# weikaolun/horovod-distributed-example

Hardware: AMD Instinct MI355X
Metric: images/sec (whole node) + scaling efficiency, ResNet-50 bf16 at 1/2/4/8 MI355X (higher is better)
Workload: dtype bf16; 1 GPU; model=ResNet-50, global_batch=2048, per_gpu_batch=2048, image=224, parallelism=dp1, optimizer=mivod FusedSGD via DistributedOptimizer, compression=none, transport=local, hip_graph=False

## Files before the change

### csrc/kernels/mv_conv.hip

```cpp
#include "mv_common.h"
#include "mv_conv.h"
#include "mv_gemm.h"

#include <algorithm>
#include <cstdlib>

namespace mv {
namespace conv {

typedef __bf16 bf16x8 __attribute__((ext_vector_type(8)));
typedef float f32x4v __attribute__((ext_vector_type(4)));
typedef uint32_t u32x2 __attribute__((ext_vector_type(2)));

constexpr int BK = 64;

__device__ __attribute__((aligned(16))) uint32_t g_zero[32];

__device__ __forceinline__ f32x4v mfma(const bf16x8& a, const bf16x8& b, const f32x4v& c) {
  return __builtin_amdgcn_mfma_f32_16x16x32_bf16(a, b, c, 0, 0, 0);
}
__device__ __forceinline__ int swz(int row, int ch) { return row * BK + ((ch ^ (row & 7)) << 3); }
__device__ __forceinline__ float round_bf16(float x) { return (float)(__bf16)x; }

__device__ __forceinline__ int remap(int bid, int nwg) {
  const int xcd = bid & 7, q = nwg >> 3, r = nwg & 7;
  const int base = xcd < r ? xcd * (q + 1) : r * (q + 1) + (xcd - r) * q;
  return base + (bid >> 3);
}

__device__ __forceinline__ void glds16(const void* src, __bf16* lds_wave_base) {
  __builtin_amdgcn_global_load_lds((const __attribute__((address_space(1))) void*)src,
                                   (__attribute__((address_space(3))) void*)lds_wave_base, 16, 0,
                                   0);
}

__device__ __forceinline__ void blds16(__amdgpu_buffer_rsrc_t rs, uint32_t off, __bf16* lds_wave_base) {
  __builtin_amdgcn_raw_ptr_buffer_load_lds(
      rs, (__attribute__((address_space(3))) void*)lds_wave_base, 16, off, 0, 0, 0);
}

struct Geo {
  int H, W, C, Ho, Wo, K, st;
  int64_t M;
  int ks = 3;
  int ph = 0, pw = 0;
  const __bf16* dy2 = nullptr;
  int k1 = 0;
  uint32_t xbytes = 0, wbytes = 0;
  int dy2x = 0;
};

template <int A_CH>
struct RowInfo {
  uint32_t addr[A_CH];
  uint32_t valid[A_CH];
};

template <int A_CH, int NT, bool DG = false>
__device__ __forceinline__ void row_info(const Geo& g, const __bf16* X, int64_t m0, int tid,
                                         int sc, RowInfo<A_CH>& ri) {
#pragma unroll
  for (int i = 0; i < A_CH; ++i) {
    const int64_t m = m0 + i * (NT / 8) + (tid >> 3);
    ri.valid[i] = 0;
    ri.addr[i] = 0;
    if (DG && m < g.M) {
      const uint32_t hw = (uint32_t)(g.Ho * g.Wo);
      const int rem = (int)((uint32_t)m % hw);
      const int ci = (int)((uint32_t)rem / (uint32_t)g.Wo), cj = rem - ci * g.Wo;
      const bool r1 = ci + 1 < g.Ho, c1 = cj + 1 < g.Wo;
      ri.valid[i] = 1u | (c1 ? 2u : 0u) | (r1 ? 4u : 0u) | (r1 && c1 ? 8u : 0u);
      ri.addr[i] = (uint32_t)((m * g.C + sc * 8) * 2);
    } else if (m < g.M) {
      const uint32_t hw = (uint32_t)(g.Ho * g.Wo), m32 = (uint32_t)m;
      const int n = (int)(m32 / hw);
      const int rem = (int)(m32 - (uint32_t)n * hw);
      const int ho = (int)((uint32_t)rem / (uint32_t)g.Wo), wo = rem - ho * g.Wo;
      const int pad = g.ks >> 1;
      const int hi0 = ho * g.st - pad, wi0 = wo * g.st - pad;
      uint32_t v = 0;
#pragma unroll
      for (int r = 0; r < 3; ++r)
#pragma unroll
        for (int s = 0; s < 3; ++s) {
          const bool ok = r < g.ks && s < g.ks && (unsigned)(hi0 + r) < (unsigned)g.H &&
                          (unsigned)(wi0 + s) < (unsigned)g.W;
          v |= (ok ? 1u : 0u) << (r * g.ks + s);
        }
      ri.valid[i] = v;
      ri.addr[i] = (uint32_t)(((((int64_t)n * g.H + hi0) * g.W + wi0) * g.C + sc * 8) * 2);
    }
  }
}

template <int N>
__device__ __forceinline__ void wait_vm() {
  asm volatile("s_waitcnt vmcnt(%0)" ::"n"(N) : "memory");
}

__device__ __forceinline__ void raw_barrier() {
  asm volatile("" ::: "memory");
  __builtin_amdgcn_s_barrier();
  asm volatile("" ::: "memory");
}

template <int BM, int BN, int WM, int WN, int EPI, int NS = 3, bool DG = false>
__global__ __launch_bounds__(WM * WN * 64)
__attribute__((amdgpu_waves_per_eu((NS == 2 && WM * WN == 8) ? 4 : 1))) void conv3x3_kernel(
    const __bf16* __restrict__ X, const __bf16* __restrict__ Wt, __bf16* __restrict__ Y, Geo g,
    int ntn, int64_t ntm, const float* __restrict__ shift, float* __restrict__ partial,
    const __bf16* __restrict__ bnx, const float* __restrict__ bnvec) {
  constexpr bool STATS = EPI != 0;
  constexpr int NT = WM * WN * 64;
  constexpr int A_CH = BM * 8 / NT;
  constexpr int WTN = BN / WN, WTM = BM / WM;
  constexpr int TN = WTN / 16, TM = WTM / 16;
  constexpr int B_CH = BN * 8 / NT;
  constexpr int LPS = A_CH + B_CH;
  constexpr int STAGE = (BM + BN) * BK;
  static_assert(NS == 2 || NS == 3, "LDS ring: 2 slots (1 stage in flight, 2 workgroups per "
                                     "CU) or 3 slots (2 stages in flight)");
  __shared__ __attribute__((aligned(16))) __bf16 smem[NS * STAGE];

  const int tid = threadIdx.x, lane = tid & 63;
  const int wid = __builtin_amdgcn_readfirstlane(tid >> 6);
  const int wm = wid / WN, wn = wid % WN;
  const int t = remap(blockIdx.x, gridDim.x);
  const int nt = t % ntn;
  const int64_t stream = t / ntn, nstreams = gridDim.x / ntn;
  const int n0 = nt * BN;
  const int taps = g.ks * g.ks;
  const int csteps = g.C / BK, KT = (DG ? (1 + g.ph) * (1 + g.pw) : taps) * csteps;
  const bool cpow2 = (csteps & (csteps - 1)) == 0;
  const int cshift = __builtin_ctz((unsigned)csteps);
  const int64_t wrow = (int64_t)taps * g.C;
  const int sc = (tid & 7) ^ ((tid >> 3) & 7);

  uint32_t brow[B_CH];
#pragma unroll
  for (int i = 0; i < B_CH; ++i)
    brow[i] = (uint32_t)(((int64_t)(n0 + i * (NT / 8) + (tid >> 3)) * wrow + sc * 8) * 2);
  const __amdgpu_buffer_rsrc_t rsX =
      __builtin_amdgcn_make_buffer_rsrc((void*)X, (short)0, (int)g.xbytes, 0x00020000);
  const __amdgpu_buffer_rsrc_t rsW =
      __builtin_amdgcn_make_buffer_rsrc((void*)Wt, (short)0, (int)g.wbytes, 0x00020000);

  auto issue = [&](const RowInfo<A_CH>& ri, int kt, int buf) {
    int tap = cpow2 ? kt >> cshift : kt / csteps;
    const int c0 = (kt - tap * csteps) * BK;
    uint32_t offa, offb;
    if constexpr (DG) {
      const int tR = g.pw ? tap >> 1 : tap, tS = g.pw ? tap & 1 : 0;
      const int rr = g.ph ? 2 * tR : 1, ss = g.pw ? 2 * tS : 1;
      offa = (uint32_t)(((tR * g.Wo + tS) * g.C + c0) * 2);
      offb = (uint32_t)(((rr * 3 + ss) * g.C + c0) * 2);
      tap = 2 * tR + tS;
    } else {
      const int r = g.ks == 3 ? (tap * 11) >> 5 : tap / g.ks;
      const int s = tap - r * g.ks;
      offa = (uint32_t)(((r * g.W + s) * g.C + c0) * 2);
      offb = (uint32_t)((tap * g.C + c0) * 2);
    }
    __bf16* As = smem + buf * STAGE;
    __bf16* Bs = As + BM * BK;
#pragma unroll
    for (int i = 0; i < A_CH; ++i) {
      const uint32_t a = ((ri.valid[i] >> tap) & 1u) ? ri.addr[i] + offa : 0xFFFFFFF0u;
      blds16(rsX, a, As + (i * NT + wid * 64) * 8);
    }
#pragma unroll
    for (int i = 0; i < B_CH; ++i)
      blds16(rsW, brow[i] + offb, Bs + (i * NT + wid * 64) * 8);
  };

  const int gq = lane >> 4, rl = lane & 15;
  float sh[EPI == 1 ? TN : 1][4], s1[TN][4], s2[TN][4];
#pragma unroll
  for (int a = 0; a < TN; ++a)
#pragma unroll
    for (int r = 0; r < 4; ++r) {
      const int col = n0 + wn * WTN + a * 16 + 4 * gq + r;
      if constexpr (EPI == 1) sh[a][r] = shift ? shift[col] : 0.f;
      s1[a][r] = 0.f;
      s2[a][r] = 0.f;
    }
  f32x4v acc[TN][TM];
#pragma unroll
  for (int a = 0; a < TN; ++a)
#pragma unroll
    for (int b = 0; b < TM; ++b) acc[a][b] = f32x4v{0.f, 0.f, 0.f, 0.f};

  int64_t mt = stream;
  if (mt < ntm) {
    RowInfo<A_CH> iri;
    row_info<A_CH, NT, DG>(g, X, mt * BM, tid, sc, iri);
    int64_t imt = mt;
    int ikt = 0;
    int islot = 0;
    issue(iri, 0, 0);
    auto issue_next = [&]() -> bool {
      int k2 = ikt + 1;
      int64_t m2 = imt;
      if (k2 == KT) { k2 = 0; m2 += nstreams; }
      if (m2 >= ntm) return false;
      if (m2 != imt) row_info<A_CH, NT, DG>(g, X, m2 * BM, tid, sc, iri);
      islot = islot + 1 == NS ? 0 : islot + 1;
      issue(iri, k2, islot);
      imt = m2;
      ikt = k2;
      return true;
    };
    bool ahead = NS == 3 ? issue_next() : false;
    int slot = 0;
    while (true) {
#pragma unroll
      for (int a = 0; a < TN; ++a)
#pragma unroll
        for (int b = 0; b < TM; ++b) acc[a][b] = f32x4v{0.f, 0.f, 0.f, 0.f};
      for (int kt = 0; kt < KT; ++kt) {
        if (NS == 3 && ahead) wait_vm<LPS>(); else wait_vm<0>();
        raw_barrier();
        ahead = issue_next();
        const __bf16* As = smem + slot * STAGE;
        const __bf16* Bs = As + BM * BK;
#pragma unroll
        for (int kk = 0; kk < BK / 32; ++kk) {
          const int ch = kk * 4 + gq;
          bf16x8 wf[TN], af[TM];
#pragma unroll
          for (int a = 0; a < TN; ++a)
            wf[a] = *reinterpret_cast<const bf16x8*>(Bs + swz(wn * WTN + a * 16 + rl, ch));
#pragma unroll
          for (int b = 0; b < TM; ++b)
            af[b] = *reinterpret_cast<const bf16x8*>(As + swz(wm * WTM + b * 16 + rl, ch));
#pragma unroll
          for (int a = 0; a < TN; ++a)
#pragma unroll
            for (int b = 0; b < TM; ++b) acc[a][b] = mfma(wf[a], af[b], acc[a][b]);
        }
        slot = slot + 1 == NS ? 0 : slot + 1;
      }
      const int64_t m0 = mt * BM;
#pragma unroll
      for (int b = 0; b < TM; ++b) {
        int64_t row = m0 + wm * WTM + b * 16 + rl;
        if (row < g.M) {
          if constexpr (DG) {
            const uint32_t hw = (uint32_t)(g.Ho * g.Wo), r32 = (uint32_t)row;
            const uint32_t n = r32 / hw, rem = r32 - n * hw;
            const uint32_t ci = rem / (uint32_t)g.Wo, cj = rem - ci * (uint32_t)g.Wo;
            row = ((int64_t)n * g.H + 2 * ci + g.ph) * g.W + 2 * cj + g.pw;
          }
#pragma unroll
          for (int a = 0; a < TN; ++a) {
            const f32x4v v = acc[a][b];
            const int col = n0 + wn * WTN + a * 16 + 4 * gq;
            if constexpr (EPI == 2) {
              const u32x2 xw = *reinterpret_cast<const u32x2*>(bnx + row * g.K + col);
              const float xv[4] = {__uint_as_float(xw[0] << 16), __uint_as_float(xw[0] & 0xffff0000u),
                                   __uint_as_float(xw[1] << 16), __uint_as_float(xw[1] & 0xffff0000u)};
              const float4 mu = *reinterpret_cast<const float4*>(bnvec + col);
              const float4 sc4 = *reinterpret_cast<const float4*>(bnvec + 2 * g.K + col);
              const float4 bi4 = *reinterpret_cast<const float4*>(bnvec + 3 * g.K + col);
              const float mus[4] = {mu.x, mu.y, mu.z, mu.w};
              const float scs[4] = {sc4.x, sc4.y, sc4.z, sc4.w};
              const float bis[4] = {bi4.x, bi4.y, bi4.z, bi4.w};
              float dv[4];
#pragma unroll
              for (int r = 0; r < 4; ++r) {
                const float d =
                    __builtin_fmaf(xv[r], scs[r], bis[r]) > 0.f ? round_bf16(v[r]) : 0.f;
                dv[r] = d;
                s1[a][r] += d;
                s2[a][r] += d * (xv[r] - mus[r]);
              }
              *reinterpret_cast<u32x2*>(Y + row * g.K + col) =
                  u32x2{cvt_pk_bf16(dv[0], dv[1]), cvt_pk_bf16(dv[2], dv[3])};
            } else {
              *reinterpret_cast<u32x2*>(Y + row * g.K + col) =
                  u32x2{cvt_pk_bf16(v[0], v[1]), cvt_pk_bf16(v[2], v[3])};
            }
            if (EPI == 1) {
#pragma unroll
              for (int r = 0; r < 4; ++r) {
                const float d = round_bf16(v[r]) - sh[a][r];
                s1[a][r] += d;
                s2[a][r] += d * d;
              }
            }
          }
        }
      }
      mt += nstreams;
      if (mt >= ntm) break;
    }
    wait_vm<0>();
    __syncthreads();
  }
  if (!STATS) return;
#pragma unroll
  for (int a = 0; a < TN; ++a)
#pragma unroll
    for (int r = 0; r < 4; ++r)
#pragma unroll
      for (int o = 1; o < 16; o <<= 1) {
        s1[a][r] += __shfl_xor(s1[a][r], o, kWave);
        s2[a][r] += __shfl_xor(s2[a][r], o, kWave);
      }
  __syncthreads();
  float* red = reinterpret_cast<float*>(smem);
  if (rl == 0) {
#pragma unroll
    for (int a = 0; a < TN; ++a)
#pragma unroll
      for (int r = 0; r < 4; ++r) {
        const int c = wn * WTN + a * 16 + 4 * gq + r;
        red[(0 * WM + wm) * BN + c] = s1[a][r];
        red[(1 * WM + wm) * BN + c] = s2[a][r];
      }
  }
  __syncthreads();
  if (stream >= ntm) return;
  for (int v = tid; v < 2 * BN; v += NT) {
    const int k = v / BN, c = v - k * BN;
    float acc_s = 0.f;
#pragma unroll
    for (int w = 0; w < WM; ++w) acc_s += red[(k * WM + w) * BN + c];
    partial[(stream * 2 + k) * g.K + n0 + c] = acc_s;
  }
}

template <int BN, bool STATS>
struct Cfg;
template <bool STATS>
struct Cfg<128, STATS> {
  static constexpr int BM = 128, WM = 2, WN = 2, NS = 2;
};
template <bool STATS>
struct Cfg<64, STATS> {
  static constexpr int BM = 256, WM = 4, WN = 2, NS = 2;
};

template <int BN, bool STATS, int EPI = STATS ? 1 : 0>
static const void* kernel_ptr() {
  using C = Cfg<BN, STATS>;
  return (const void*)&conv3x3_kernel<C::BM, BN, C::WM, C::WN, EPI, C::NS>;
}

template <int BN, bool STATS>
static int64_t streams_for(int64_t ntm, int ntn) {
  static int per = [] {
    int v = 0;
    if (hipOccupancyMaxActiveBlocksPerMultiprocessor(
            &v, kernel_ptr<BN, STATS>(), Cfg<BN, STATS>::WM * Cfg<BN, STATS>::WN * 64, 0) !=
            hipSuccess || v < 1)
      v = 1;
    return v;
  }();
  static int cus = [] {
    int dev = 0, v = 0;
    if (hipGetDevice(&dev) != hipSuccess ||
        hipDeviceGetAttribute(&v, hipDeviceAttributeMultiprocessorCount, dev) != hipSuccess || v < 1)
      v = 256;
    return v;
  }();
  int64_t s = (int64_t)cus * per / ntn;
  s = std::max<int64_t>(1, std::min(s, ntm));
  return s;
}

}
}

static int conv_bn_of(int K) { return K % 128 == 0 ? 128 : 64; }

static bool conv256_route(int K) { return K % 256 == 0 && K <= 2048; }

int64_t mv_conv3x3_partials(int64_t M, int K) {
  using namespace mv::conv;
  if (conv256_route(K)) return mv_gemm256_partials(M, K);
  if (conv_bn_of(K) == 128)
    return streams_for<128, true>((M + Cfg<128, true>::BM - 1) / Cfg<128, true>::BM, K / 128);
  return streams_for<64, true>((M + Cfg<64, true>::BM - 1) / Cfg<64, true>::BM, K / 64);
}

bool mv_conv3x3(const void* x, const void* w, void* y, int N, int H, int W, int C, int K,
                int stride, const float* shift, float* partial, hipStream_t st,
                const void* bn_x, const float* bn_vec) {
  return mv_conv_nhwc(x, w, y, N, H, W, C, K, 3, stride, shift, partial, st, bn_x, bn_vec);
}

bool mv_conv_nhwc(const void* x, const void* w, void* y, int N, int H, int W, int C, int K, int ks,
                  int stride, const float* shift, float* partial, hipStream_t st,
                  const void* bn_x, const float* bn_vec, const float* in_scale,
                  const float* in_bias) {
  using namespace mv::conv;
  if (C % 64 != 0 || K % 64 != 0 || (stride != 1 && stride != 2) || (ks != 1 && ks != 3))
    return false;
  if ((int64_t)N * H * W >= (int64_t(1) << 31)) return false;
  const bool bna = in_scale != nullptr;
  if (mv_conv64_supported(N, H, W, C, K, ks, stride)) {
    const int64_t M = (int64_t)N * H * W;
    int grid = partial ? (int)mv_conv3x3_partials(M, K) : 0;
    if (!partial) {
      int dev = 0, cus = 0;
      if (hipGetDevice(&dev) != hipSuccess ||
          hipDeviceGetAttribute(&cus, hipDeviceAttributeMultiprocessorCount, dev) != hipSuccess ||
          cus < 1)
        cus = 256;
      grid = cus;
    }
    return mv_conv64(x, w, y, N, H, W, shift, partial, grid, st, bn_x, bn_vec, in_scale,
                     in_bias);
  }
  if (bna) return false;
  if (conv256_route(K))
    return mv_conv256(x, w, y, N, H, W, C, K, ks, stride, shift, partial, bn_x, bn_vec, st);
  Geo g;
  g.ks = ks;
  g.H = H;
  g.W = W;
  g.C = C;
  g.K = K;
  g.st = stride;
  g.Ho = (H - 1) / stride + 1;
  g.Wo = (W - 1) / stride + 1;
  g.M = (int64_t)N * g.Ho * g.Wo;
  if ((int64_t)N * H * W * C * 2 >= (int64_t(1) << 32) - 16 ||
      (int64_t)K * ks * ks * C * 2 >= (int64_t(1) << 32) - 16)
    return false;
  g.xbytes = (uint32_t)((int64_t)N * H * W * C * 2);
  g.wbytes = (uint32_t)((int64_t)K * ks * ks * C * 2);
  const __bf16* X = (const __bf16*)x;
  const __bf16* Wt = (const __bf16*)w;
  __bf16* Y = (__bf16*)y;
  const __bf16* BX = (const __bf16*)bn_x;
  if (bn_x && !partial) return false;
#define MV_LAUNCH(BNV, ST)                                                                     \
  {                                                                                            \
    constexpr int BMV = Cfg<BNV, ST>::BM, WMV = Cfg<BNV, ST>::WM, WNV = Cfg<BNV, ST>::WN;      \
    constexpr int NSV = Cfg<BNV, ST>::NS;                                                      \
    const int64_t ntm = (g.M + BMV - 1) / BMV;                                                 \
    const int ntn = K / BNV;                                                                   \
    const int64_t ns = streams_for<BNV, ST>(ntm, ntn);                                         \
    if (BX)                                                                                    \
      hipLaunchKernelGGL((conv3x3_kernel<BMV, BNV, WMV, WNV, 2, NSV>), dim3((unsigned)(ns * ntn)),\
                         dim3(WMV * WNV * 64), 0, st, X, Wt, Y, g, ntn, ntm, shift, partial, BX, \
                         bn_vec);                                                              \
    else                                                                                       \
      hipLaunchKernelGGL((conv3x3_kernel<BMV, BNV, WMV, WNV, ST ? 1 : 0, NSV>),                  \
                         dim3((unsigned)(ns * ntn)), dim3(WMV * WNV * 64), 0, st, X, Wt, Y, g,   \
                         ntn, ntm, shift, partial, BX, bn_vec);                                \
  }
  if (conv_bn_of(K) == 128) {
    if (partial) MV_LAUNCH(128, true) else MV_LAUNCH(128, false)
  } else {
    if (partial) MV_LAUNCH(64, true) else MV_LAUNCH(64, false)
  }
#undef MV_LAUNCH
  return true;
}

namespace mv {
namespace conv {
struct TfTensor {
  const __bf16* src;
  __bf16* dst;
  int K, C, ks;
};
struct TfBlock {
  int t, tap, k0, c0;
};
__global__ __launch_bounds__(256) void transpose_filters_kernel(const TfTensor* __restrict__ ts,
                                                                const TfBlock* __restrict__ bl) {
  __shared__ __attribute__((aligned(16))) __bf16 tile[64][72];
  const TfBlock b = bl[blockIdx.x];
  const TfTensor tt = ts[b.t];
  const int ks = tt.ks, taps = ks * ks;
  const int r = b.tap / ks, s = b.tap - r * ks;
  const int ftap = (ks - 1 - r) * ks + (ks - 1 - s);
  typedef __bf16 bf16x8t __attribute__((ext_vector_type(8)));
  if (b.k0 + 64 <= tt.K && b.c0 + 64 <= tt.C && (tt.C & 7) == 0 && (tt.K & 7) == 0) {
    const int lr = threadIdx.x >> 3, l8 = (threadIdx.x & 7) * 8;
#pragma unroll
    for (int h = 0; h < 2; ++h) {
      const int i = lr + 32 * h;
      *reinterpret_cast<bf16x8t*>(&tile[i][l8]) = *reinterpret_cast<const bf16x8t*>(
          tt.src + ((int64_t)(b.k0 + i) * taps + ftap) * tt.C + b.c0 + l8);
    }
    __syncthreads();
#pragma unroll
    for (int h = 0; h < 2; ++h) {
      const int i = lr + 32 * h;
      bf16x8t v;
#pragma unroll
      for (int j = 0; j < 8; ++j) v[j] = tile[l8 + j][i];
      *reinterpret_cast<bf16x8t*>(tt.dst + ((int64_t)(b.c0 + i) * taps + b.tap) * tt.K + b.k0 +
                                  l8) = v;
    }
    return;
  }
  const int tx = threadIdx.x & 63, ty = threadIdx.x >> 6;
  for (int i = ty; i < 64; i += 4) {
    const int k = b.k0 + i, c = b.c0 + tx;
    tile[i][tx] = (k < tt.K && c < tt.C) ? tt.src[((int64_t)k * taps + ftap) * tt.C + c]
                                         : (__bf16)0.f;
  }
  __syncthreads();
  for (int i = ty; i < 64; i += 4) {
    const int c = b.c0 + i, k = b.k0 + tx;
    if (c < tt.C && k < tt.K) tt.dst[((int64_t)c * taps + b.tap) * tt.K + k] = tile[tx][i];
  }
}
}
}

int64_t mv_transpose_filters_blocks(const int* K, const int* C, const int* ks, int n) {
  int64_t nb = 0;
  for (int i = 0; i < n; ++i)
    nb += (int64_t)ks[i] * ks[i] * ((K[i] + 63) / 64) * ((C[i] + 63) / 64);
  return nb;
}

void mv_transpose_filters_table(const void* const* src, void* const* dst, const int* K,
                                const int* C, const int* ks, int n, void* host_image) {
  using namespace mv::conv;
  TfTensor* ts = reinterpret_cast<TfTensor*>(host_image);
  TfBlock* bl = reinterpret_cast<TfBlock*>(ts + n);
  int64_t j = 0;
  for (int i = 0; i < n; ++i) {
    ts[i] = TfTensor{(const __bf16*)src[i], (__bf16*)dst[i], K[i], C[i], ks[i]};
    for (int tap = 0; tap < ks[i] * ks[i]; ++tap)
      for (int k0 = 0; k0 < K[i]; k0 += 64)
        for (int c0 = 0; c0 < C[i]; c0 += 64) bl[j++] = TfBlock{i, tap, k0, c0};
  }
}

int64_t mv_transpose_filters_table_bytes(int n, int64_t blocks) {
  return (int64_t)n * (int64_t)sizeof(mv::conv::TfTensor) + blocks * (int64_t)sizeof(mv::conv::TfBlock);
}

void mv_transpose_filters(const void* table, int n, int64_t blocks, hipStream_t st) {
  using namespace mv::conv;
  const TfTensor* ts = reinterpret_cast<const TfTensor*>(table);
  const TfBlock* bl = reinterpret_cast<const TfBlock*>(ts + n);
  hipLaunchKernelGGL(transpose_filters_kernel, dim3((unsigned)blocks), dim3(256), 0, st, ts, bl);
}

bool mv_conv3x3_s2_dgrad_supported(int Nb, int H, int W, int C, int K) {
  if (mv_dgrad256_s2_supported(Nb, H, W, C, K)) return true;
  return Nb > 0 && H >= 2 && W >= 2 && !(H & 1) && !(W & 1) && C % 64 == 0 && K % 64 == 0 &&
         C > 0 && K > 0 && (int64_t)Nb * (H / 2) * (W / 2) * K * 2 < (int64_t(1) << 32) - 16 &&
         (int64_t)C * 9 * K * 2 < (int64_t(1) << 32) - 16 && (int64_t)Nb * H * W < (int64_t(1) << 31);
}

bool mv_conv3x3_s2_dgrad(const void* dy, const void* wt, void* dx, int Nb, int H, int W, int C,
                         int K, hipStream_t st) {
  using namespace mv::conv;
  if (mv_dgrad256_s2_supported(Nb, H, W, C, K))
    return mv_dgrad256_s2(dy, wt, dx, Nb, H, W, C, K, st);
  if (!mv_conv3x3_s2_dgrad_supported(Nb, H, W, C, K)) return false;
  Geo g;
  g.ks = 3;
  g.st = 2;
  g.H = H;
  g.W = W;
  g.C = K;
  g.K = C;
  g.Ho = H / 2;
  g.Wo = W / 2;
  g.M = (int64_t)Nb * g.Ho * g.Wo;
  g.xbytes = (uint32_t)(g.M * K * 2);
  g.wbytes = (uint32_t)((int64_t)C * 9 * K * 2);
  const __bf16* X = (const __bf16*)dy;
  const __bf16* Wt = (const __bf16*)wt;
  __bf16* Y = (__bf16*)dx;
#define MV_LAUNCH_DG(BNV)                                                                      \
  {                                                                                            \
    constexpr int BMV = Cfg<BNV, false>::BM, WMV = Cfg<BNV, false>::WM;                        \
    constexpr int WNV = Cfg<BNV, false>::WN, NSV = Cfg<BNV, false>::NS;                        \
    const int64_t ntm = (g.M + BMV - 1) / BMV;                                                 \
    const int ntn = C / BNV;                                                                   \
    const int64_t ns = streams_for<BNV, false>(ntm, ntn);                                      \
    hipLaunchKernelGGL((conv3x3_kernel<BMV, BNV, WMV, WNV, 0, NSV, true>),                      \
                       dim3((unsigned)(ns * ntn)), dim3(WMV * WNV * 64), 0, st, X, Wt, Y, g, ntn, \
                       ntm, nullptr, nullptr, nullptr, nullptr);                               \
  }
  for (int c = 3; c >= 0; --c) {
    g.ph = c >> 1;
    g.pw = c & 1;
    if (conv_bn_of(C) == 128) MV_LAUNCH_DG(128) else MV_LAUNCH_DG(64)
  }
#undef MV_LAUNCH_DG
  return true;
}

namespace mv {
// ... 542 lines not shown
```

### csrc/kernels/mv_conv64.hip

```cpp
#include "mv_common.h"
#include "mv_conv.h"

#include <type_traits>

namespace mv {
namespace conv64 {

typedef __bf16 bf16x8 __attribute__((ext_vector_type(8)));
typedef float f32x4v __attribute__((ext_vector_type(4)));
typedef uint32_t u32x2 __attribute__((ext_vector_type(2)));
typedef uint32_t u32x4 __attribute__((ext_vector_type(4)));

constexpr int kC = 64;
constexpr int kR = 8;
constexpr int kPR = kR + 2;
constexpr int kPW = 64;
constexpr int kThreads = 512;
constexpr int kTMW = 7;
constexpr int kTN = 2;
constexpr int kMaxW = kPW - 2;
constexpr int kMT = 4 * kTMW;
constexpr int kFilt = kC * 9 * kC;
constexpr int kPatchChunks = kPR * kPW * 8;
constexpr int kLoads = (kPatchChunks + kThreads - 1) / kThreads;

__device__ __forceinline__ f32x4v mfma(const bf16x8& a, const bf16x8& b, const f32x4v& c) {
  return __builtin_amdgcn_mfma_f32_16x16x32_bf16(a, b, c, 0, 0, 0);
}
__device__ __forceinline__ int fidx(int k, int tap, int c) {
  return ((k * 9 + tap) * 8 + (c ^ (k & 7))) * 8;
}
__device__ __forceinline__ int pidx(int row, int col, int c) {
  return ((row * kPW + col) * 8 + (c ^ (col & 7))) * 8;
}
__device__ __forceinline__ float round_bf16(float x) { return (float)(__bf16)x; }

struct Geo64 {
  int N, H, W;
  int hblocks;
  int64_t tiles;
};

__device__ __forceinline__ void bn_relu8(u32x4& v, const float (&sc)[8], const float (&bi)[8]) {
  uint32_t w[4] = {v[0], v[1], v[2], v[3]};
#pragma unroll
  for (int j = 0; j < 4; ++j) {
    const float lo = fmaxf(__builtin_fmaf(__uint_as_float(w[j] << 16), sc[2 * j], bi[2 * j]), 0.f);
    const float hi =
        fmaxf(__builtin_fmaf(__uint_as_float(w[j] & 0xffff0000u), sc[2 * j + 1], bi[2 * j + 1]), 0.f);
    w[j] = cvt_pk_bf16(lo, hi);
  }
  v = u32x4{w[0], w[1], w[2], w[3]};
}

template <int EPI>
__global__ __launch_bounds__(kThreads, 1) __attribute__((amdgpu_waves_per_eu(2, 2))) void conv64_kernel(
    const __bf16* __restrict__ X, const __bf16* __restrict__ Wt, __bf16* __restrict__ Y,
    Geo64 g, const float* __restrict__ shift, float* __restrict__ partial,
    const __bf16* __restrict__ bnx, const float* __restrict__ bnvec,
    const float* __restrict__ xsc, const float* __restrict__ xbi) {
  __shared__ __attribute__((aligned(16))) __bf16 lds[kFilt + kPR * kPW * kC];
  __bf16* fs = lds;
  __bf16* ps = lds + kFilt;
  const int tid = threadIdx.x, lane = tid & 63;
  const int wv = __builtin_amdgcn_readfirstlane(tid >> 6);
  const int nh = wv & 1, mg = wv >> 1;
  const int gq = lane >> 4, rl = lane & 15;
  const int W = g.W, H = g.H;

  for (int q = tid; q < kC * 9 * 8; q += kThreads) {
    const int k = q / 72, rem = q - k * 72, tap = rem >> 3, c = rem & 7;
    *reinterpret_cast<u32x4*>(fs + fidx(k, tap, c)) =
        *reinterpret_cast<const u32x4*>(Wt + (int64_t)q * 8);
  }

  int pbase[kTMW], pcol[kTMW];
#pragma unroll
  for (int b = 0; b < kTMW; ++b) {
    const int p = (mg * kTMW + b) * 16 + rl;
    const int r = p / W, c = p - r * W;
    const bool ok = r < kR;
    pbase[b] = ok ? (r * kPW + c) * 64 : 0;
    pcol[b] = ok ? c : 0;
  }

  static_assert(kThreads == 8 * kPW && kLoads == kPR, "one patch row per load");
  const int scol = tid >> 3, sch = tid & 7;
  const bool colok = scol >= 1 && scol - 1 < W;
  const int64_t coff = (int64_t)(scol - 1) * kC + sch * 8;
  const int soff = pidx(0, scol, sch);
  const bool bna = EPI != 2 && xsc != nullptr;
  float asc[8], abi[8];
#pragma unroll
  for (int j = 0; j < 8; ++j) {
    asc[j] = bna ? xsc[sch * 8 + j] : 0.f;
    abi[j] = bna ? xbi[sch * 8 + j] : 0.f;
  }
  u32x4 pre[kLoads];
  auto gload = [&](int64_t t) {
    const int n = (int)(t / g.hblocks), h0 = (int)(t - (int64_t)n * g.hblocks) * kR;
    const __bf16* img = X + (int64_t)n * H * W * kC;
#pragma unroll
    for (int i = 0; i < kLoads; ++i) {
      const int ih = h0 + i - 1;
      u32x4 v = {0u, 0u, 0u, 0u};
      if (colok && ih >= 0 && ih < H)
        v = *reinterpret_cast<const u32x4*>(img + (int64_t)ih * W * kC + coff);
      pre[i] = v;
    }
  };

  float s1[kTN][4], s2[kTN][4];
#pragma unroll
  for (int a = 0; a < kTN; ++a)
#pragma unroll
    for (int r = 0; r < 4; ++r) {
      s1[a][r] = 0.f;
      s2[a][r] = 0.f;
    }

  f32x4v acc[kTN][kTMW];
  auto epilogue = [&](int64_t tp) {
    const float* shp = shift;
    const float* bvp = bnvec;
    asm volatile("" : "+s"(shp));
    asm volatile("" : "+s"(bvp));
    const int n = (int)(tp / g.hblocks), h0 = (int)(tp - (int64_t)n * g.hblocks) * kR;
    float4 cv[EPI == 0 ? 1 : kTN][EPI == 2 ? 3 : 1];
    if constexpr (EPI != 0) {
#pragma unroll
      for (int a = 0; a < kTN; ++a) {
        const int col = nh * 32 + a * 16 + 4 * gq;
        if constexpr (EPI == 1) {
          cv[a][0] = shp ? *reinterpret_cast<const float4*>(shp + col) : float4{0.f, 0.f, 0.f, 0.f};
        } else {
          cv[a][0] = *reinterpret_cast<const float4*>(bvp + col);
          cv[a][1] = *reinterpret_cast<const float4*>(bvp + 2 * kC + col);
          cv[a][2] = *reinterpret_cast<const float4*>(bvp + 3 * kC + col);
        }
      }
    }
    const __bf16* ximg = bnx + (EPI == 2 ? (int64_t)n * H * W * kC : 0);
    __bf16* yimg = Y + (int64_t)n * H * W * kC;
    auto half = [&](auto b0c, auto b1c) {
      constexpr int B0 = decltype(b0c)::value, B1 = decltype(b1c)::value;
      int off[B1 - B0];
      bool ok[B1 - B0];
#pragma unroll
      for (int b = B0; b < B1; ++b) {
        const int p = (mg * kTMW + b) * 16 + rl;
        const int r = p / W;
        ok[b - B0] = r < kR && h0 + r < H;
        off[b - B0] = ((h0 + r) * W + (p - r * W)) * kC;
      }
      u32x2 xw[EPI == 2 ? B1 - B0 : 1][EPI == 2 ? kTN : 1];
      if constexpr (EPI == 2) {
#pragma unroll
        for (int b = B0; b < B1; ++b)
#pragma unroll
          for (int a = 0; a < kTN; ++a)
            xw[b - B0][a] = ok[b - B0] ? *reinterpret_cast<const u32x2*>(
                                             ximg + off[b - B0] + nh * 32 + a * 16 + 4 * gq)
                                       : u32x2{0u, 0u};
      }
#pragma unroll
      for (int b = B0; b < B1; ++b) {
        if (!ok[b - B0]) continue;
#pragma unroll
        for (int a = 0; a < kTN; ++a) {
          const f32x4v v = acc[a][b];
          const int col = nh * 32 + a * 16 + 4 * gq;
          __bf16* yp = yimg + off[b - B0] + col;
          if constexpr (EPI == 2) {
            const u32x2 x2 = xw[b - B0][a];
            const float xv[4] = {__uint_as_float(x2[0] << 16), __uint_as_float(x2[0] & 0xffff0000u),
                                 __uint_as_float(x2[1] << 16), __uint_as_float(x2[1] & 0xffff0000u)};
            const float mus[4] = {cv[a][0].x, cv[a][0].y, cv[a][0].z, cv[a][0].w};
            const float scs[4] = {cv[a][1].x, cv[a][1].y, cv[a][1].z, cv[a][1].w};
            const float bis[4] = {cv[a][2].x, cv[a][2].y, cv[a][2].z, cv[a][2].w};
            float dv[4];
#pragma unroll
            for (int r = 0; r < 4; ++r) {
              const float d = __builtin_fmaf(xv[r], scs[r], bis[r]) > 0.f ? round_bf16(v[r]) : 0.f;
              dv[r] = d;
              s1[a][r] += d;
              s2[a][r] += d * (xv[r] - mus[r]);
            }
            *reinterpret_cast<u32x2*>(yp) =
                u32x2{cvt_pk_bf16_cc(dv[0], dv[1]), cvt_pk_bf16_cc(dv[2], dv[3])};
          } else {
            const uint32_t lo = cvt_pk_bf16_cc(v[0], v[1]), hi = cvt_pk_bf16_cc(v[2], v[3]);
            *reinterpret_cast<u32x2*>(yp) = u32x2{lo, hi};
            if constexpr (EPI == 1) {
              const float vb[4] = {__uint_as_float(lo << 16), __uint_as_float(lo & 0xffff0000u),
                                   __uint_as_float(hi << 16), __uint_as_float(hi & 0xffff0000u)};
              const float shs[4] = {cv[a][0].x, cv[a][0].y, cv[a][0].z, cv[a][0].w};
#pragma unroll
              for (int r = 0; r < 4; ++r) {
                const float d = vb[r] - shs[r];
                s1[a][r] += d;
                s2[a][r] += d * d;
              }
            }
          }
        }
      }
    };
    half(std::integral_constant<int, 0>{}, std::integral_constant<int, 4>{});
    half(std::integral_constant<int, 4>{}, std::integral_constant<int, kTMW>{});
  };
  auto frags = [&](int step, bf16x8 (&wf)[kTN], bf16x8 (&xf)[kTMW]) {
    const int tap = step >> 1, ch = (step & 1) * 4 + gq;
    const int dr = tap / 3, dc = tap - dr * 3;
    const int off = dr * kPW * 64 + dc * 64;
#pragma unroll
    for (int a = 0; a < kTN; ++a)
      wf[a] = *reinterpret_cast<const bf16x8*>(fs + fidx(nh * 32 + a * 16 + rl, tap, ch));
#pragma unroll
    for (int b = 0; b < kTMW; ++b)
      xf[b] = *reinterpret_cast<const bf16x8*>(
          ps + pbase[b] + off + ((ch ^ ((pcol[b] + dc) & 7)) << 3));
  };
  auto mmas = [&](const bf16x8 (&wf)[kTN], const bf16x8 (&xf)[kTMW]) {
#pragma unroll
    for (int a = 0; a < kTN; ++a)
#pragma unroll
      for (int b = 0; b < kTMW; ++b) acc[a][b] = mfma(wf[a], xf[b], acc[a][b]);
  };

  auto bn_stage = [&](int64_t tt) {
    const int h0 = (int)(tt - (tt / g.hblocks) * g.hblocks) * kR;
#pragma unroll
    for (int i = 0; i < kLoads; ++i) {
      const int ih = h0 + i - 1;
      if (colok && ih >= 0 && ih < H) bn_relu8(pre[i], asc, abi);
    }
  };
  int64_t t = blockIdx.x;
  int64_t tprev = -1;
  if (t < g.tiles) {
    gload(t);
    if (bna) bn_stage(t);
  }
  for (; t < g.tiles; t += gridDim.x) {
    __syncthreads();
#pragma unroll
    for (int i = 0; i < kLoads; ++i)
      *reinterpret_cast<u32x4*>(ps + soff + i * kPW * 64) = pre[i];
    __syncthreads();
    if (tprev >= 0) epilogue(tprev);
    __builtin_amdgcn_sched_barrier(0);
    if (t + gridDim.x < g.tiles) gload(t + gridDim.x);
    __builtin_amdgcn_sched_barrier(0);

#pragma unroll
    for (int a = 0; a < kTN; ++a)
#pragma unroll
      for (int b = 0; b < kTMW; ++b) acc[a][b] = f32x4v{0.f, 0.f, 0.f, 0.f};
#pragma unroll
    for (int st = 0; st < 18; ++st) {
      bf16x8 wA[kTN], xA[kTMW];
      frags(st, wA, xA);
      mmas(wA, xA);
      __builtin_amdgcn_sched_barrier(0);
      if (st == 8 && bna && t + gridDim.x < g.tiles) {
        bn_stage(t + gridDim.x);
        __builtin_amdgcn_sched_barrier(0);
      }
    }
    tprev = t;
  }
  if (tprev >= 0) epilogue(tprev);
  if constexpr (EPI == 0) return;
#pragma unroll
  for (int a = 0; a < kTN; ++a)
#pragma unroll
    for (int r = 0; r < 4; ++r)
#pragma unroll
      for (int o = 1; o < 16; o <<= 1) {
        s1[a][r] += __shfl_xor(s1[a][r], o, kWave);
        s2[a][r] += __shfl_xor(s2[a][r], o, kWave);
      }
  __syncthreads();
  float* red = reinterpret_cast<float*>(ps);
  if (rl == 0) {
#pragma unroll
    for (int a = 0; a < kTN; ++a)
#pragma unroll
      for (int r = 0; r < 4; ++r) {
        const int c = nh * 32 + a * 16 + 4 * gq + r;
        red[(0 * 4 + mg) * kC + c] = s1[a][r];
        red[(1 * 4 + mg) * kC + c] = s2[a][r];
      }
  }
  __syncthreads();
  for (int v = tid; v < 2 * kC; v += kThreads) {
    const int k = v / kC, c = v - k * kC;
    float s = 0.f;
#pragma unroll
    for (int m = 0; m < 4; ++m) s += red[(k * 4 + m) * kC + c];
    partial[((int64_t)blockIdx.x * 2 + k) * kC + c] = s;
  }
}

}
}

bool mv_conv64_supported(int N, int H, int W, int C, int K, int ks, int stride) {
  return N > 0 && C == 64 && K == 64 && ks == 3 && stride == 1 && H >= 1 && W >= 1 &&
         (int64_t)H * W * 64 < (int64_t(1) << 31) &&
         W <= mv::conv64::kMaxW && (int64_t)mv::conv64::kR * W <= 16 * mv::conv64::kMT;
}

bool mv_conv64(const void* x, const void* w, void* y, int N, int H, int W, const float* shift,
               float* partial, int grid, hipStream_t st, const void* bn_x, const float* bn_vec,
               const float* in_scale, const float* in_bias) {
  using namespace mv::conv64;
  if (!mv_conv64_supported(N, H, W, 64, 64, 3, 1) || grid < 1) return false;
  Geo64 g;
  g.N = N;
  g.H = H;
  g.W = W;
  g.hblocks = (H + kR - 1) / kR;
  g.tiles = (int64_t)N * g.hblocks;
  const __bf16* X = (const __bf16*)x;
  const __bf16* Wt = (const __bf16*)w;
  __bf16* Y = (__bf16*)y;
  if ((in_scale == nullptr) != (in_bias == nullptr) || (bn_x && in_scale)) return false;
  if (bn_x) {
    if (!partial) return false;
    hipLaunchKernelGGL(conv64_kernel<2>, dim3(grid), dim3(kThreads), 0, st, X, Wt, Y, g,
                       nullptr, partial, (const __bf16*)bn_x, bn_vec, in_scale, in_bias);
  } else if (partial) {
    hipLaunchKernelGGL(conv64_kernel<1>, dim3(grid), dim3(kThreads), 0, st, X, Wt, Y, g,
                       shift, partial, nullptr, nullptr, in_scale, in_bias);
  } else {
    hipLaunchKernelGGL(conv64_kernel<0>, dim3(grid), dim3(kThreads), 0, st, X, Wt, Y, g,
                       nullptr, nullptr, nullptr, nullptr, in_scale, in_bias);
  }
  return true;
}

namespace mv {
namespace conv64 {

typedef short s16x4 __attribute__((ext_vector_type(4)));

constexpr int kWThreads = 512;
constexpr int kDyPix = kR * 56;
constexpr int kWLoadsDy = kDyPix * 8 / kWThreads;
constexpr int kWLoadsX = kPR;

__device__ __forceinline__ int dswz(int p) { return ((p >> 1) & 3) << 1; }
constexpr int kPS = 80;
constexpr int kPC = 58;

__device__ __forceinline__ bf16x8 tr8p(const __bf16* pa, const __bf16* pb) {
  const s16x4 a = __builtin_amdgcn_ds_read_tr16_b64_v4i16((__attribute__((address_space(3))) s16x4*)pa);
  const s16x4 b = __builtin_amdgcn_ds_read_tr16_b64_v4i16((__attribute__((address_space(3))) s16x4*)pb);
  typedef short s16x8 __attribute__((ext_vector_type(8)));
  const s16x8 o = __builtin_shufflevector(a, b, 0, 1, 2, 3, 4, 5, 6, 7);
  return __builtin_bit_cast(bf16x8, o);
}

__global__ __launch_bounds__(kWThreads, 1) __attribute__((amdgpu_waves_per_eu(2, 2)))
void wgrad64_kernel(const __bf16* __restrict__ X, const __bf16* __restrict__ DY,
                    float* __restrict__ partial, Geo64 g, const float* __restrict__ xsc,
                    const float* __restrict__ xbi) {
  __shared__ __attribute__((aligned(16))) __bf16 lds[kDyPix * kC + kPR * kPC * kPS];
  __bf16* ds = lds;
  __bf16* ps = lds + kDyPix * kC;
  const int tid = threadIdx.x, lane = tid & 63;
  const int wv = __builtin_amdgcn_readfirstlane(tid >> 6);
  const int ct = wv & 3, kh = wv >> 2;
  const int gq = lane >> 4, cl = lane & 15;
  const int W = g.W, H = g.H;
  const int npix = kR * W;

  const int sch = tid & 7, spix = tid >> 3;
  const bool colok = spix >= 1 && spix - 1 < W;
  const int64_t xcoff = (int64_t)(spix - 1) * kC + sch * 8;
  const bool bna = xsc != nullptr;
  float asc[8], abi[8];
#pragma unroll
  for (int j = 0; j < 8; ++j) {
    asc[j] = bna ? xsc[sch * 8 + j] : 0.f;
    abi[j] = bna ? xbi[sch * 8 + j] : 0.f;
  }
  u32x4 pdy[kWLoadsDy], px[kWLoadsX];
  auto gload = [&](int64_t t) {
    const int n = (int)(t / g.hblocks), h0 = (int)(t - (int64_t)n * g.hblocks) * kR;
    const __bf16* img = X + (int64_t)n * H * W * kC;
#pragma unroll
    for (int i = 0; i < kWLoadsX; ++i) {
      const int ih = h0 + i - 1;
      u32x4 v = {0u, 0u, 0u, 0u};
      if (colok && ih >= 0 && ih < H)
        v = *reinterpret_cast<const u32x4*>(img + (int64_t)ih * W * kC + xcoff);
      px[i] = v;
    }
    const __bf16* dimg = DY + (int64_t)n * H * W * kC;
#pragma unroll
    for (int i = 0; i < kWLoadsDy; ++i) {
      const int p = spix + 64 * i;
      const int r = p / W;
      u32x4 v = {0u, 0u, 0u, 0u};
      if (p < npix && h0 + r < H)
        v = *reinterpret_cast<const u32x4*>(dimg + ((int64_t)(h0 + r) * W + (p - r * W)) * kC +
                                            sch * 8);
      pdy[i] = v;
    }
  };

  const __bf16* ads[2][2];
#pragma unroll
  for (int u = 0; u < 2; ++u)
#pragma unroll
    for (int h = 0; h < 2; ++h) {
      const int r = 4 * gq + 16 * h + (cl >> 2), e = 16 * (2 * kh + u) + 4 * (cl & 3);
      ads[u][h] = ds + r * 64 + (((e >> 3) ^ dswz(r)) << 3) + (e & 7);
    }
  const __bf16* pbase = ps + (cl >> 2) * kPS + 16 * ct + 4 * (cl & 3);
  f32x4v acc[2][9];
#pragma unroll
  for (int u = 0; u < 2; ++u)
#pragma unroll
    for (int tp = 0; tp < 9; ++tp) acc[u][tp] = f32x4v{0.f, 0.f, 0.f, 0.f};

  auto bn_stage = [&](int64_t tt) {
    const int h0 = (int)(tt - (tt / g.hblocks) * g.hblocks) * kR;
#pragma unroll
    for (int i = 0; i < kWLoadsX; ++i) {
      const int ih = h0 + i - 1;
      if (colok && ih >= 0 && ih < H) bn_relu8(px[i], asc, abi);
    }
  };
  int64_t t = blockIdx.x;
  if (t < g.tiles) gload(t);
  for (; t < g.tiles; t += gridDim.x) {
    __syncthreads();
    if (bna) bn_stage(t);
    if (spix < kPC) {
#pragma unroll
      for (int i = 0; i < kWLoadsX; ++i)
        *reinterpret_cast<u32x4*>(ps + (i * kPC + spix) * kPS + sch * 8) = px[i];
    }
#pragma unroll
    for (int i = 0; i < kWLoadsDy; ++i) {
      const int p = spix + 64 * i;
      *reinterpret_cast<u32x4*>(ds + p * 64 + ((sch ^ dswz(p)) << 3)) = pdy[i];
    }
    __syncthreads();
    if (t + gridDim.x < g.tiles) gload(t + gridDim.x);
    __builtin_amdgcn_sched_barrier(0);
    const int nks = (npix + 31) >> 5;
    int ra = (4 * gq) / W, ca = 4 * gq - ra * W;
    int rb = (4 * gq + 16) / W, cb = 4 * gq + 16 - rb * W;
#pragma unroll 1
    for (int ks = 0; ks < nks; ++ks) {
      const int pa = ks * 32 + 4 * gq;
      const int qa = pa < npix ? ra * kPC + ca : 0;
      const int qb = pa + 16 < npix ? rb * kPC + cb : 0;
      bf16x8 af[2];
#pragma unroll
      for (int u = 0; u < 2; ++u) af[u] = tr8p(ads[u][0] + ks * 32 * 64, ads[u][1] + ks * 32 * 64);
      const __bf16* ba = pbase + qa * kPS;
      const __bf16* bb = pbase + qb * kPS;
#pragma unroll
      for (int tp = 0; tp < 9; ++tp) {
        const int off = ((tp / 3) * kPC + tp % 3) * kPS;
        const bf16x8 bfr = tr8p(ba + off, bb + off);
#pragma unroll
        for (int u = 0; u < 2; ++u) acc[u][tp] = mfma(af[u], bfr, acc[u][tp]);
      }
      __builtin_amdgcn_sched_barrier(0);
      ca += 32;
      while (ca >= W) {
        ca -= W;
        ++ra;
      }
      cb += 32;
      while (cb >= W) {
        cb -= W;
        ++rb;
      }
    }
  }
  float* pp = partial + (int64_t)blockIdx.x * 9 * kC * kC;
#pragma unroll
  for (int tp = 0; tp < 9; ++tp)
#pragma unroll
    for (int u = 0; u < 2; ++u)
#pragma unroll
      for (int r = 0; r < 4; ++r) {
        const int k = 16 * (2 * kh + u) + 4 * gq + r, c = 16 * ct + cl;
        pp[((int64_t)tp * kC + k) * kC + c] = acc[u][tp][r];
      }
}

}
}

bool mv_wgrad64_supported(int N, int H, int W, int C, int K, int stride) {
  return N > 0 && C == 64 && K == 64 && stride == 1 && H >= 1 && W >= 4 && W % 4 == 0 &&
         W <= 56 && (int64_t)H * W * 64 < (int64_t(1) << 31);
}

bool mv_wgrad64(const void* x, const void* dy, float* partial, int grid, int N, int H, int W,
                hipStream_t st, const float* in_scale, const float* in_bias) {
  using namespace mv::conv64;
  if (!mv_wgrad64_supported(N, H, W, 64, 64, 1) || grid < 1) return false;
  Geo64 g;
  g.N = N;
  g.H = H;
  g.W = W;
  g.hblocks = (H + kR - 1) / kR;
  g.tiles = (int64_t)N * g.hblocks;
  if ((in_scale == nullptr) != (in_bias == nullptr)) return false;
  hipLaunchKernelGGL(wgrad64_kernel, dim3(grid), dim3(kWThreads), 0, st, (const __bf16*)x,
                     (const __bf16*)dy, partial, g, in_scale, in_bias);
  return true;
}
```

Before: 18680 images/sec.

## Incrementally advance conv row coordinates and prefetch residual epilogue loads early

The 3x3 conv kernel now keeps each row's (n, ho, wo) position and moves it forward by a precomputed step when the tile changes, instead of redoing integer divisions per tile. It also builds the padding validity mask with bit operations, and the EPI==1 stats now reuse the packed bf16 values rather than rounding again. The 64-channel conv issues part of the EPI==2 residual-input loads before the barrier and the rest at the start of the epilogue, so that global load latency overlaps other work. In exchange, registers holding row positions and early-loaded values stay live for longer, which may raise register pressure.

New measurement: 18790 images/sec, median of 6. About the same (+0.6%).

```diff
diff --git a/csrc/kernels/mv_conv.hip b/csrc/kernels/mv_conv.hip
--- a/csrc/kernels/mv_conv.hip
+++ b/csrc/kernels/mv_conv.hip
@@ -56,40 +56,75 @@
   uint32_t valid[A_CH];
 };
 
+template <int R>
+struct RowPos {
+  uint32_t n[R], ho[R], wo[R];
+};
+struct RowStep {
+  uint32_t dn, dho, dwo;
+};
+
+__device__ __forceinline__ RowStep row_step(const Geo& g, int64_t rows) {
+  const uint32_t hw = (uint32_t)(g.Ho * g.Wo), d = (uint32_t)rows;
+  RowStep s;
+  s.dn = d / hw;
+  const uint32_t rem = d - s.dn * hw;
+  s.dho = rem / (uint32_t)g.Wo;
+  s.dwo = rem - s.dho * (uint32_t)g.Wo;
+  return s;
+}
+
+template <int R>
+__device__ __forceinline__ void row_pos_init(const Geo& g, int64_t first, int stride,
+                                             RowPos<R>& p) {
+  const uint32_t hw = (uint32_t)(g.Ho * g.Wo);
+#pragma unroll
+  for (int i = 0; i < R; ++i) {
+    const int64_t m = first + i * stride;
+    const uint32_t m32 = m < g.M ? (uint32_t)m : 0u;
+    p.n[i] = m32 / hw;
+    const uint32_t rem = m32 - p.n[i] * hw;
+    p.ho[i] = rem / (uint32_t)g.Wo;
+    p.wo[i] = rem - p.ho[i] * (uint32_t)g.Wo;
+  }
+}
+
+template <int R>
+__device__ __forceinline__ void row_pos_advance(const Geo& g, const RowStep& s, RowPos<R>& p) {
+#pragma unroll
+  for (int i = 0; i < R; ++i) {
+    uint32_t wo = p.wo[i] + s.dwo;
+    const bool cw = wo >= (uint32_t)g.Wo;
+    p.wo[i] = cw ? wo - (uint32_t)g.Wo : wo;
+    uint32_t ho = p.ho[i] + s.dho + (cw ? 1u : 0u);
+    const bool chh = ho >= (uint32_t)g.Ho;
+    p.ho[i] = chh ? ho - (uint32_t)g.Ho : ho;
+    p.n[i] += s.dn + (chh ? 1u : 0u);
+  }
+}
+
 template <int A_CH, int NT, bool DG = false>
-__device__ __forceinline__ void row_info(const Geo& g, const __bf16* X, int64_t m0, int tid,
-                                         int sc, RowInfo<A_CH>& ri) {
+__device__ __forceinline__ void row_info(const Geo& g, int64_t m0, int tid, int sc,
+                                         const RowPos<A_CH>& p, RowInfo<A_CH>& ri) {
 #pragma unroll
   for (int i = 0; i < A_CH; ++i) {
     const int64_t m = m0 + i * (NT / 8) + (tid >> 3);
-    ri.valid[i] = 0;
-    ri.addr[i] = 0;
-    if (DG && m < g.M) {
-      const uint32_t hw = (uint32_t)(g.Ho * g.Wo);
-      const int rem = (int)((uint32_t)m % hw);
-      const int ci = (int)((uint32_t)rem / (uint32_t)g.Wo), cj = rem - ci * g.Wo;
-      const bool r1 = ci + 1 < g.Ho, c1 = cj + 1 < g.Wo;
-      ri.valid[i] = 1u | (c1 ? 2u : 0u) | (r1 ? 4u : 0u) | (r1 && c1 ? 8u : 0u);
-      ri.addr[i] = (uint32_t)((m * g.C + sc * 8) * 2);
-    } else if (m < g.M) {
-      const uint32_t hw = (uint32_t)(g.Ho * g.Wo), m32 = (uint32_t)m;
-      const int n = (int)(m32 / hw);
-      const int rem = (int)(m32 - (uint32_t)n * hw);
-      const int ho = (int)((uint32_t)rem / (uint32_t)g.Wo), wo = rem - ho * g.Wo;
+    const bool in = m < g.M;
+    uint32_t v, addr;
+    if constexpr (DG) {
+      const bool r1 = p.ho[i] + 1u < (uint32_t)g.Ho, c1 = p.wo[i] + 1u < (uint32_t)g.Wo;
+      v = 1u | (c1 ? 2u : 0u) | (r1 ? 4u : 0u) | (r1 && c1 ? 8u : 0u);
+      addr = ((uint32_t)m * (uint32_t)g.C + (uint32_t)(sc * 8)) * 2u;
+    } else {
       const int pad = g.ks >> 1;
-      const int hi0 = ho * g.st - pad, wi0 = wo * g.st - pad;
-      uint32_t v = 0;
-#pragma unroll
-      for (int r = 0; r < 3; ++r)
-#pragma unroll
-        for (int s = 0; s < 3; ++s) {
-          const bool ok = r < g.ks && s < g.ks && (unsigned)(hi0 + r) < (unsigned)g.H &&
-                          (unsigned)(wi0 + s) < (unsigned)g.W;
-          v |= (ok ? 1u : 0u) << (r * g.ks + s);
-        }
-      ri.valid[i] = v;
-      ri.addr[i] = (uint32_t)(((((int64_t)n * g.H + hi0) * g.W + wi0) * g.C + sc * 8) * 2);
-    }
+      const int hi0 = (int)p.ho[i] * g.st - pad, wi0 = (int)p.wo[i] * g.st - pad;
+      const uint32_t cb = (wi0 >= 0 ? 1u : 0u) | 2u | (wi0 + 2 < g.W ? 4u : 0u);
+      v = g.ks == 3 ? ((hi0 >= 0 ? cb : 0u) | (cb << 3) | (hi0 + 2 < g.H ? cb << 6 : 0u)) : 1u;
+      addr = (((p.n[i] * (uint32_t)g.H + (uint32_t)hi0) * (uint32_t)g.W + (uint32_t)wi0) *
+                  (uint32_t)g.C + (uint32_t)(sc * 8)) * 2u;
+    }
+    ri.valid[i] = in ? v : 0u;
+    ri.addr[i] = in ? addr : 0u;
   }
 }
 
@@ -192,8 +227,13 @@
 
   int64_t mt = stream;
   if (mt < ntm) {
+    const RowStep tstep = row_step(g, nstreams * BM);
+    RowPos<A_CH> ipos;
+    row_pos_init<A_CH>(g, mt * BM + (tid >> 3), NT / 8, ipos);
     RowInfo<A_CH> iri;
-    row_info<A_CH, NT, DG>(g, X, mt * BM, tid, sc, iri);
+    row_info<A_CH, NT, DG>(g, mt * BM, tid, sc, ipos, iri);
+    [[maybe_unused]] RowPos<DG ? TM : 1> opos;
+    if constexpr (DG) row_pos_init<TM>(g, mt * BM + wm * WTM + (lane & 15), 16, opos);
     int64_t imt = mt;
     int ikt = 0;
     int islot = 0;
@@ -203,7 +243,10 @@
       int64_t m2 = imt;
       if (k2 == KT) { k2 = 0; m2 += nstreams; }
       if (m2 >= ntm) return false;
-      if (m2 != imt) row_info<A_CH, NT, DG>(g, X, m2 * BM, tid, sc, iri);
+      if (m2 != imt) {
+        row_pos_advance<A_CH>(g, tstep, ipos);
+        row_info<A_CH, NT, DG>(g, m2 * BM, tid, sc, ipos, iri);
+      }
       islot = islot + 1 == NS ? 0 : islot + 1;
       issue(iri, k2, islot);
       imt = m2;
@@ -245,12 +288,8 @@
       for (int b = 0; b < TM; ++b) {
         int64_t row = m0 + wm * WTM + b * 16 + rl;
         if (row < g.M) {
-          if constexpr (DG) {
-            const uint32_t hw = (uint32_t)(g.Ho * g.Wo), r32 = (uint32_t)row;
-            const uint32_t n = r32 / hw, rem = r32 - n * hw;
-            const uint32_t ci = rem / (uint32_t)g.Wo, cj = rem - ci * (uint32_t)g.Wo;
-            row = ((int64_t)n * g.H + 2 * ci + g.ph) * g.W + 2 * cj + g.pw;
-          }
+          if constexpr (DG)
+            row = ((int64_t)opos.n[b] * g.H + 2 * opos.ho[b] + g.ph) * g.W + 2 * opos.wo[b] + g.pw;
 #pragma unroll
           for (int a = 0; a < TN; ++a) {
             const f32x4v v = acc[a][b];
@@ -277,15 +316,17 @@
               *reinterpret_cast<u32x2*>(Y + row * g.K + col) =
                   u32x2{cvt_pk_bf16(dv[0], dv[1]), cvt_pk_bf16(dv[2], dv[3])};
             } else {
-              *reinterpret_cast<u32x2*>(Y + row * g.K + col) =
-                  u32x2{cvt_pk_bf16(v[0], v[1]), cvt_pk_bf16(v[2], v[3])};
-            }
-            if (EPI == 1) {
-#pragma unroll
-              for (int r = 0; r < 4; ++r) {
-                const float d = round_bf16(v[r]) - sh[a][r];
-                s1[a][r] += d;
-                s2[a][r] += d * d;
+              const uint32_t lo = cvt_pk_bf16(v[0], v[1]), hi = cvt_pk_bf16(v[2], v[3]);
+              *reinterpret_cast<u32x2*>(Y + row * g.K + col) = u32x2{lo, hi};
+              if constexpr (EPI == 1) {
+                const float vb[4] = {__uint_as_float(lo << 16), __uint_as_float(lo & 0xffff0000u),
+                                     __uint_as_float(hi << 16), __uint_as_float(hi & 0xffff0000u)};
+#pragma unroll
+                for (int r = 0; r < 4; ++r) {
+                  const float d = vb[r] - sh[a][r];
+                  s1[a][r] += d;
+                  s2[a][r] += d * d;
+                }
               }
             }
           }
@@ -293,6 +334,7 @@
       }
       mt += nstreams;
       if (mt >= ntm) break;
+      if constexpr (DG) row_pos_advance<TM>(g, tstep, opos);
     }
     wait_vm<0>();
     __syncthreads();
diff --git a/csrc/kernels/mv_conv64.hip b/csrc/kernels/mv_conv64.hip
--- a/csrc/kernels/mv_conv64.hip
+++ b/csrc/kernels/mv_conv64.hip
@@ -120,6 +120,30 @@
     }
 
   f32x4v acc[kTN][kTMW];
+  constexpr int kEarly = 4;
+  u32x2 exw[EPI == 2 ? kTMW : 1][EPI == 2 ? kTN : 1];
+  auto epi_load = [&](int64_t tp, auto b0c, auto b1c) {
+    constexpr int B0 = decltype(b0c)::value, B1 = decltype(b1c)::value;
+    if constexpr (EPI == 2) {
+      const int n = (int)(tp / g.hblocks), h0 = (int)(tp - (int64_t)n * g.hblocks) * kR;
+      const __bf16* ximg = bnx + (int64_t)n * H * W * kC;
+#pragma unroll
+      for (int b = B0; b < B1; ++b) {
+        const int p = (mg * kTMW + b) * 16 + rl;
+        const int r = pbase[b] >> 12;
+        const bool ok = p < kR * W && h0 + r < H;
+        const int off = ((h0 + r) * W + pcol[b]) * kC;
+#pragma unroll
+        for (int a = 0; a < kTN; ++a)
+          exw[b][a] = ok ? *reinterpret_cast<const u32x2*>(ximg + off + nh * 32 + a * 16 + 4 * gq)
+                         : u32x2{0u, 0u};
+      }
+    }
+  };
+  static_assert(kPW * 64 == 4096, "row from pbase >> 12");
+  const std::integral_constant<int, 0> kB0{};
+  const std::integral_constant<int, kEarly> kB1{};
+  const std::integral_constant<int, kTMW> kB2{};
   auto epilogue = [&](int64_t tp) {
     const float* shp = shift;
     const float* bvp = bnvec;
@@ -127,6 +151,7 @@
     asm volatile("" : "+s"(bvp));
     const int n = (int)(tp / g.hblocks), h0 = (int)(tp - (int64_t)n * g.hblocks) * kR;
     float4 cv[EPI == 0 ? 1 : kTN][EPI == 2 ? 3 : 1];
+    epi_load(tp, kB1, kB2);
     if constexpr (EPI != 0) {
 #pragma unroll
       for (int a = 0; a < kTN; ++a) {
@@ -140,7 +165,6 @@
         }
       }
     }
-    const __bf16* ximg = bnx + (EPI == 2 ? (int64_t)n * H * W * kC : 0);
     __bf16* yimg = Y + (int64_t)n * H * W * kC;
     auto half = [&](auto b0c, auto b1c) {
       constexpr int B0 = decltype(b0c)::value, B1 = decltype(b1c)::value;
@@ -149,19 +173,9 @@
 #pragma unroll
       for (int b = B0; b < B1; ++b) {
         const int p = (mg * kTMW + b) * 16 + rl;
-        const int r = p / W;
-        ok[b - B0] = r < kR && h0 + r < H;
-        off[b - B0] = ((h0 + r) * W + (p - r * W)) * kC;
-      }
-      u32x2 xw[EPI == 2 ? B1 - B0 : 1][EPI == 2 ? kTN : 1];
-      if constexpr (EPI == 2) {
-#pragma unroll
-        for (int b = B0; b < B1; ++b)
-#pragma unroll
-          for (int a = 0; a < kTN; ++a)
-            xw[b - B0][a] = ok[b - B0] ? *reinterpret_cast<const u32x2*>(
-                                             ximg + off[b - B0] + nh * 32 + a * 16 + 4 * gq)
-                                       : u32x2{0u, 0u};
+        const int r = pbase[b] >> 12;
+        ok[b - B0] = p < kR * W && h0 + r < H;
+        off[b - B0] = ((h0 + r) * W + pcol[b]) * kC;
       }
 #pragma unroll
       for (int b = B0; b < B1; ++b) {
@@ -172,7 +186,7 @@
           const int col = nh * 32 + a * 16 + 4 * gq;
           __bf16* yp = yimg + off[b - B0] + col;
           if constexpr (EPI == 2) {
-            const u32x2 x2 = xw[b - B0][a];
+            const u32x2 x2 = exw[b][a];
             const float xv[4] = {__uint_as_float(x2[0] << 16), __uint_as_float(x2[0] & 0xffff0000u),
                                  __uint_as_float(x2[1] << 16), __uint_as_float(x2[1] & 0xffff0000u)};
             const float mus[4] = {cv[a][0].x, cv[a][0].y, cv[a][0].z, cv[a][0].w};
@@ -243,6 +257,10 @@
     if (bna) bn_stage(t);
   }
   for (; t < g.tiles; t += gridDim.x) {
+    if constexpr (EPI == 2) {
+      if (tprev >= 0) epi_load(tprev, kB0, kB1);
+      __builtin_amdgcn_sched_barrier(0);
+    }
     __syncthreads();
 #pragma unroll
     for (int i = 0; i < kLoads; ++i)
@@ -270,7 +288,10 @@
     }
     tprev = t;
   }
-  if (tprev >= 0) epilogue(tprev);
+  if (tprev >= 0) {
+    epi_load(tprev, kB0, kB1);
+    epilogue(tprev);
+  }
   if constexpr (EPI == 0) return;
 #pragma unroll
   for (int a = 0; a < kTN; ++a)
```
